# AliaksandrSiarohin/wc-gan

Hardware: AMD Instinct MI355X
Metric: images/sec G+D step, CIFAR-10 ResNet-SN+WC, batch 64 (higher is better)
Workload: dtype f32; 1 GPU; CIFAR-10 ResNet SN uncond + WC (scripts/cifar10_resnet_sn_uncond.sh), batch 64/GPU, training_ratio 5, generator_batch_multiple 2; parallelism=dp1, wc_statistics=per-replica, launch=hipgraph

## Files before the change

include/wc_hip.h:

```cpp
#ifndef WC_HIP_H
#define WC_HIP_H

#include <stddef.h>
#include <stdint.h>

#ifdef __cplusplus
extern "C" {
#endif

#define WC_ABI_VERSION 8

#define WC_OK                 0
#define WC_ERR_NULL          -1
#define WC_ERR_SHAPE         -2
#define WC_ERR_CHANNELS      -3
#define WC_ERR_WORKSPACE     -4
#define WC_ERR_ARG           -5

typedef void* wc_stream_t;

int         wc_abi_version(void);
const char* wc_error_string(int code);

#define WC_CORE_API "wc_stats_f32 wc_factor_f64 wc_color_f32 wc_group_bias_f32 wc_apply_f32 wc_apply_act_f32 " \
// ... 246 lines not shown

#define WC_CONV_HIST_FLOATS (4 * 512 + 16)
#define WC_CONV_HIST_REDO (4 * 512)
int wc_conv_split_hist_f32(const float* x, int64_t n, int relu, void* hi, void* lo, float* scale, float* colsum_partials , int C,
                           float* hist, int bootstrap, wc_stream_t stream);

int wc_conv_split_leaky_f32(const float* x, int64_t n, float negative_slope, void* hi, void* lo, float* scale, void* amax_scratch,
                            float* colsum_partials , int C, wc_stream_t stream);
int wc_conv_split_hist_leaky_f32(const float* x, int64_t n, float negative_slope, void* hi, void* lo, float* scale,
                                 float* colsum_partials , int C, float* hist, int bootstrap, wc_stream_t stream);
int wc_conv_leaky_bwd_f32(float* dx, const float* x, int64_t n, float negative_slope, wc_stream_t stream);

size_t wc_conv_weights_bytes(const wc_conv_geom* g);
int wc_conv_weights_f32(const float* w, int64_t stride_k, int64_t stride_n, int64_t stride_r, int64_t stride_s,
                        int64_t n_elems, const wc_conv_geom* g, void* image, float* scale, void* amax_scratch,
                        const float* known_amax, int known_count, wc_stream_t stream);

int wc_conv_weights_pair_f32(const float* w, int64_t stride_r, int64_t stride_s, int64_t n_elems,
                             int64_t a_stride_k, int64_t a_stride_n, const wc_conv_geom* ga, void* image_a,
                             int64_t b_stride_k, int64_t b_stride_n, const wc_conv_geom* gb, void* image_b,
                             float* scale, void* amax_scratch, const float* known_amax, int known_count,
                             wc_stream_t stream);

size_t wc_conv_workspace_bytes(const wc_conv_geom* g);
int wc_conv_f16x3(const void* xhi, const void* xlo, const float* xscale, const void* wimage, const float* wscale,
                  const float* bias, const void* zero_line, const wc_conv_geom* g, int relu, float* y,
                  void* ws, size_t ws_bytes, wc_stream_t stream);

int wc_conv_res_supported(const wc_conv_geom* g);
int wc_conv_res_f16x3(const void* xhi, const void* xlo, const float* xscale, const void* wimage, const float* wscale,
                      const float* bias, const float* res, const void* zero_line, const wc_conv_geom* g, float* y,
                      void* ws, size_t ws_bytes, wc_stream_t stream);
int wc_conv_block_dx_f32(const float* dx1, const float* x, const float* other, int64_t N, int64_t H, int64_t W, int C, int down,
                         float* out, wc_stream_t stream);

size_t wc_conv_wrw_workspace_bytes(const wc_conv_geom* g);
int wc_conv_wrw_f16x3(const void* xhi, const void* xlo, const float* xscale, const void* ghi, const void* glo,
                      const float* gscale, const void* zero_line, const wc_conv_geom* g, float* dw, int64_t stride_k,
                      int64_t stride_n, int64_t stride_r, int64_t stride_s, void* ws, size_t ws_bytes,
                      wc_stream_t stream);

int    wc_conv_wrw_narrow_supported(int64_t N, int64_t H, int64_t W, int Cin, int Cout, int ksize);
size_t wc_conv_wrw_narrow_workspace_bytes(int64_t N, int64_t H, int64_t W, int Cin, int Cout, int ksize);
int    wc_conv_wrw_narrow_f32(const float* x, const float* gy, int64_t N, int64_t H, int64_t W, int Cin, int Cout, int ksize,
                              float* dw, int64_t stride_k, int64_t stride_n, int64_t stride_r, int64_t stride_s, float* db ,
                              void* ws, size_t ws_bytes, wc_stream_t stream);
// ... 118 lines not shown
```

wc_gan_amd/_lib.py:

```python
from __future__ import annotations

import ctypes
import os
from ctypes import c_float, c_char_p, c_double, c_int, c_int64, c_size_t, c_void_p

_HERE = os.path.dirname(os.path.abspath(__file__))
LIB_PATH = os.path.join(_HERE, "libwc_hip.so")

WC_OK = 0
ABI_VERSION = 8
ERRORS = {-1: "WC_ERR_NULL", -2: "WC_ERR_SHAPE", -3: "WC_ERR_CHANNELS", -4: "WC_ERR_WORKSPACE", -5: "WC_ERR_ARG"}

SIGNATURES = {
    "wc_abi_version": (c_int, []),
    "wc_error_string": (c_char_p, [c_int]),
    "wc_stats_workspace_bytes": (c_size_t, [c_int64, c_int, c_int]),
    "wc_factor_workspace_bytes": (c_size_t, [c_int, c_int]),
    "wc_color_workspace_bytes": (c_size_t, [c_int, c_int]),
    "wc_bwd_reduce_workspace_bytes": (c_size_t, [c_int64, c_int64, c_int, c_int, c_int]),
    "wc_bwd_factor_workspace_bytes": (c_size_t, [c_int, c_int]),
    "wc_apply_workspace_bytes": (c_size_t, [c_int64, c_int64, c_int, c_int]),
    "wc_apply_plan_bytes": (c_size_t, [c_int, c_int]),
    "wc_bwd_apply_workspace_bytes": (c_size_t, [c_int64, c_int64, c_int, c_int]),
    "wc_stats_f32": (c_int, [c_void_p, c_int64, c_int, c_int, c_void_p, c_void_p, c_void_p, c_size_t, c_void_p]),
# ... 102 lines not shown
    "wc_conv_weights_f32": (c_int, [c_void_p, c_int64, c_int64, c_int64, c_int64, c_int64, c_void_p, c_void_p, c_void_p,
                                    c_void_p, c_void_p, c_int, c_void_p]),
    "wc_spectral_norm_amax_offset": (c_size_t, [c_int, c_int]),
    "wc_spectral_norm_error_offset": (c_size_t, [c_int, c_int]),
    "wc_conv_split_hist_f32": (c_int, [c_void_p, c_int64, c_int, c_void_p, c_void_p, c_void_p, c_void_p, c_int, c_void_p, c_int, c_void_p]),
    "wc_conv_split_leaky_f32": (c_int, [c_void_p, c_int64, c_float, c_void_p, c_void_p, c_void_p, c_void_p, c_void_p, c_int, c_void_p]),
    "wc_conv_split_hist_leaky_f32": (c_int, [c_void_p, c_int64, c_float, c_void_p, c_void_p, c_void_p, c_void_p, c_int, c_void_p, c_int, c_void_p]),
    "wc_conv_leaky_bwd_f32": (c_int, [c_void_p, c_void_p, c_int64, c_float, c_void_p]),
    "wc_conv_narrow64_supported": (c_int, [c_int64, c_int64, c_int64, c_int, c_int, c_int]),
    "wc_conv_wrw_narrow64_workspace_bytes": (c_size_t, [c_int64, c_int64, c_int64, c_int, c_int, c_int]),
    "wc_conv_wrw_narrow64_f32": (c_int, [c_void_p, c_void_p, c_int64, c_int64, c_int64, c_int, c_int, c_int, c_void_p, c_int64, c_int64, c_int64,
                                         c_int64, c_void_p, c_void_p, c_size_t, c_void_p]),
    "wc_conv_fwd_narrow_f32": (c_int, [c_void_p, c_void_p, c_int64, c_int64, c_int64, c_int64, c_void_p, c_int64, c_int64, c_int64, c_int, c_int, c_int,
                                       c_int, c_void_p, c_void_p]),
    "wc_conv_wrw_narrow_supported": (c_int, [c_int64, c_int64, c_int64, c_int, c_int, c_int]),
    "wc_conv_wrw_narrow_workspace_bytes": (c_size_t, [c_int64, c_int64, c_int64, c_int, c_int, c_int]),
    "wc_conv_wrw_narrow_f32": (c_int, [c_void_p, c_void_p, c_int64, c_int64, c_int64, c_int, c_int, c_int, c_void_p, c_int64, c_int64, c_int64,
                                       c_int64, c_void_p, c_void_p, c_size_t, c_void_p]),
    "wc_conv_split_colsum_f32": (c_int, [c_void_p, c_int64, c_int, c_void_p, c_void_p, c_void_p, c_void_p, c_void_p, c_int, c_void_p]),
    "wc_conv_wrw_bias_f16x3": (c_int, [c_void_p, c_void_p, c_void_p, c_void_p, c_void_p, c_void_p, c_void_p, c_void_p, c_void_p,
                                       c_int64, c_int64, c_int64, c_int64, c_void_p, c_void_p, c_void_p, c_size_t, c_void_p]),
    "wc_conv_weights_pair_f32": (c_int, [c_void_p, c_int64, c_int64, c_int64, c_int64, c_int64, c_void_p, c_void_p,
                                         c_int64, c_int64, c_void_p, c_void_p, c_void_p, c_void_p, c_void_p, c_int, c_void_p]),
    "wc_conv_wrw_workspace_bytes": (c_size_t, [c_void_p]),
    "wc_conv_wrw_f16x3": (c_int, [c_void_p, c_void_p, c_void_p, c_void_p, c_void_p, c_void_p, c_void_p, c_void_p, c_void_p,
                                  c_int64, c_int64, c_int64, c_int64, c_void_p, c_size_t, c_void_p]),
    "wc_conv_workspace_bytes": (c_size_t, [c_void_p]),
    "wc_conv_f16x3": (c_int, [c_void_p, c_void_p, c_void_p, c_void_p, c_void_p, c_void_p, c_void_p, c_void_p, c_int,
                              c_void_p, c_void_p, c_size_t, c_void_p]),
    "wc_conv_bwd_pair_supported": (c_int, [c_void_p, c_void_p]),
    "wc_conv_bwd_pair_workspace_bytes": (c_size_t, [c_void_p, c_void_p]),
    "wc_conv_bwd_pair_f16x3": (c_int, [c_void_p, c_void_p, c_void_p, c_void_p, c_void_p, c_void_p, c_void_p, c_void_p, c_void_p, c_size_t,
                                       c_void_p, c_void_p, c_void_p, c_void_p, c_void_p, c_int64, c_int64, c_int64, c_int64,
                                       c_void_p, c_void_p, c_void_p, c_size_t, c_void_p]),
    "wc_std_stats_workspace_bytes": (c_size_t, [c_int64, c_int, c_int]),
    "wc_std_stats_f32": (c_int, [c_void_p, c_int64, c_int, c_int, c_void_p, c_void_p, c_void_p, c_size_t, c_void_p]),
    "wc_std_factor_f64": (c_int, [c_void_p, c_void_p, c_int64, c_int, c_int, c_double, c_double, c_int, c_int, c_void_p, c_void_p,
                                  c_void_p, c_void_p, c_int, c_void_p, c_void_p, c_void_p, c_void_p, c_void_p]),
    "wc_std_apply_f32": (c_int, [c_void_p, c_void_p, c_void_p, c_void_p, c_int64, c_int64, c_int, c_int, c_int, c_void_p, c_void_p]),
    "wc_std_bwd_reduce_workspace_bytes": (c_size_t, [c_int64, c_int64, c_int, c_int]),
    "wc_std_bwd_reduce_f32": (c_int, [c_void_p, c_void_p, c_void_p, c_void_p, c_void_p, c_int64, c_int64, c_int, c_int, c_int,
                                      c_void_p, c_void_p, c_void_p, c_size_t, c_void_p]),
    "wc_std_bwd_factor_f64": (c_int, [c_void_p, c_void_p, c_void_p, c_void_p, c_void_p, c_int64, c_int, c_int, c_int,
                                      c_void_p, c_void_p, c_void_p, c_void_p, c_void_p]),
    "wc_std_bwd_apply_f32": (c_int, [c_void_p, c_void_p, c_void_p, c_void_p, c_void_p, c_void_p, c_void_p, c_int64, c_int64, c_int, c_int,
                                     c_int, c_void_p, c_void_p]),
# ... 37 lines not shown


class SnItem(ctypes.Structure):
    _fields_ = [("W", c_void_p), ("u", c_void_p), ("v", c_void_p), ("w_sn", c_void_p), ("sigma", c_void_p),
                ("u_used", c_void_p), ("v_used", c_void_p), ("ws", c_void_p), ("rows", c_int), ("cols", c_int)]


class SnBwdItem(ctypes.Structure):
    _fields_ = [("g", c_void_p), ("w_sn", c_void_p), ("u", c_void_p), ("v", c_void_p), ("sigma", c_void_p),
                ("dW", c_void_p), ("ws", c_void_p), ("rows", c_int), ("cols", c_int)]


class ConvGeom(ctypes.Structure):
    _fields_ = [("N", c_int), ("H", c_int), ("W", c_int), ("Hin", c_int), ("Win", c_int), ("Cin", c_int),
                ("Hout", c_int), ("Wout", c_int), ("Cout", c_int), ("in_stride", c_int), ("out_stride", c_int),
                ("ntaps", c_int), ("nphase", c_int),
                ("dy", (ctypes.c_byte * 16) * 4), ("dx", (ctypes.c_byte * 16) * 4),
                ("off_y", ctypes.c_byte * 4), ("off_x", ctypes.c_byte * 4),
                ("nsrc", (ctypes.c_byte * 16) * 4),
                ("wr", ((ctypes.c_byte * 4) * 16) * 4), ("ws", ((ctypes.c_byte * 4) * 16) * 4),
                ("wcoef", c_float)]


_lib = None


class WcHipError(RuntimeError):
    pass


def shared_gpu_guard(device_count=None) -> bool:
    if "WC_K2_TWO_LAUNCH" in os.environ:
        if os.environ["WC_K2_TWO_LAUNCH"] == "0":
            del os.environ["WC_K2_TWO_LAUNCH"]
        return False
    try:
        ranks = int(os.environ.get("LOCAL_WORLD_SIZE", "1") or 1)
    except ValueError:
        ranks = 1
    if ranks <= 1:
        return False
    if any(os.environ.get(k) for k in ("HIP_VISIBLE_DEVICES", "CUDA_VISIBLE_DEVICES", "ROCR_VISIBLE_DEVICES")):
        return False
    if device_count is None:
        try:
            import torch
# ... 38 lines not shown
```

wc_gan_amd/conv.py:

```python
from __future__ import annotations

import ctypes
import os

import torch
import torch.nn.functional as F

from . import _lib, _state
from .ops import _ptr, _stream

_zero_lines = {}


def _zero_line(device):
    z = _zero_lines.get(device)
    if z is None:
        z = _zero_lines[device] = torch.zeros(64, dtype=torch.uint8, device=device)
    return z


def _plain(r, s):
    return [(r, s)], 1.0


# ... 201 lines not shown
def block_input_gradient(dx1, x, other, down):
    N, H, W, C = dx1.shape
    want = (N, H // 2, W // 2, C) if down else (N, H, W, C)
    if not (dx1.is_contiguous() and x.is_contiguous() and other.is_contiguous() and x.shape == dx1.shape and tuple(other.shape) == want
            and dx1.dtype == x.dtype == other.dtype == torch.float32):
        raise ValueError("block_input_gradient: dense fp32 NHWC tensors, `other` of dx1's shape (at half resolution when down)")
    out = torch.empty_like(dx1)
    _lib.check(_lib.load().wc_conv_block_dx_f32(_ptr(dx1), _ptr(x), _ptr(other), N, H, W, C, 1 if down else 0, _ptr(out), _stream()),
               "wc_conv_block_dx_f32")
    return out


def leaky_backward_(dx, x, slope):
    if not (dx.is_contiguous() and x.is_contiguous() and dx.shape == x.shape and dx.dtype == x.dtype == torch.float32):
        raise ValueError("leaky_backward_: dense fp32 tensors of one shape")
    _lib.check(_lib.load().wc_conv_leaky_bwd_f32(_ptr(dx), _ptr(x), dx.numel(), float(slope), _stream()), "wc_conv_leaky_bwd_f32")
    return dx


def _storage_extent(w):
    return 1 + sum((n - 1) * s for n, s in zip(w.shape, w.stride()))


def weight_image(w, geom, k_axis, n_axis):
    lib = _lib.load()
    nbytes = lib.wc_conv_weights_bytes(ctypes.addressof(geom))
    img = torch.empty(nbytes, dtype=torch.uint8, device=w.device)
    scale = torch.empty(1 + 512, dtype=torch.float32, device=w.device)
    ext = _storage_extent(w)
    if ext != w.numel():
        raise ValueError("weight must be dense")
    known = getattr(w, '_wc_amax', None)
    _lib.check(lib.wc_conv_weights_f32(_ptr(w), w.stride(k_axis), w.stride(n_axis), w.stride(2), w.stride(3), ext,
                                       ctypes.addressof(geom), _ptr(img), _ptr(scale), scale.data_ptr() + 4,
                                       _ptr(known), 0 if known is None else known.numel(), _stream()),
               "wc_conv_weights_f32")
    return img, scale


def weight_image_pair(w, fwd, bwd):
    lib = _lib.load()
    (ga, ka, na), (gb, kb, nb) = fwd, bwd
    img_a = torch.empty(lib.wc_conv_weights_bytes(ctypes.addressof(ga)), dtype=torch.uint8, device=w.device)
    img_b = torch.empty(lib.wc_conv_weights_bytes(ctypes.addressof(gb)), dtype=torch.uint8, device=w.device)
    scale = torch.empty(2 + 512, dtype=torch.float32, device=w.device)
    ext = _storage_extent(w)
    if ext != w.numel():
        raise ValueError("weight must be dense")
    known = getattr(w, '_wc_amax', None)
    _lib.check(lib.wc_conv_weights_pair_f32(_ptr(w), w.stride(2), w.stride(3), ext,
                                            w.stride(ka), w.stride(na), ctypes.addressof(ga), _ptr(img_a),
                                            w.stride(kb), w.stride(nb), ctypes.addressof(gb), _ptr(img_b),
                                            _ptr(scale), scale.data_ptr() + 8, _ptr(known), 0 if known is None else known.numel(),
                                            _stream()), "wc_conv_weights_pair_f32")
    return (img_a, scale[0:1]), (img_b, scale[1:2])


def _cached_image(w, key, geom, k_axis, n_axis):
    return weight_image(w, geom, k_axis, n_axis)


def run(planes, image, geom, bias=None, relu=False, nbytes=None, res=None):
    hi, lo, xs = planes
    img, ws = image
    lib = _lib.load()
    y = torch.empty((geom.N, geom.Hout, geom.Wout, geom.Cout), dtype=torch.float32, device=hi.device)
    if nbytes is None:
        nbytes = lib.wc_conv_workspace_bytes(ctypes.addressof(geom))
    work = torch.empty(nbytes, dtype=torch.uint8, device=hi.device) if nbytes else None
    if res is not None:
        if relu or not (res.is_contiguous() and res.shape == y.shape and res.dtype == torch.float32 and res.device == y.device):
            raise ValueError("run: the residual is a dense fp32 tensor of the output's shape (and there is no ReLU behind it)")
        _lib.check(lib.wc_conv_res_f16x3(_ptr(hi), _ptr(lo), _ptr(xs), _ptr(img), _ptr(ws), _ptr(bias) if bias is not None else None,
                                         _ptr(res), _ptr(_zero_line(hi.device)), ctypes.addressof(geom), _ptr(y),
                                         _ptr(work), nbytes, _stream()), "wc_conv_res_f16x3")
        return y
    _lib.check(lib.wc_conv_f16x3(_ptr(hi), _ptr(lo), _ptr(xs), _ptr(img), _ptr(ws), _ptr(bias) if bias is not None else None,
                                 _ptr(_zero_line(hi.device)), ctypes.addressof(geom), 1 if relu else 0, _ptr(y),
                                 _ptr(work), nbytes, _stream()), "wc_conv_f16x3")
    return y


# ... 58 lines not shown
                                          _ptr(work_dx), plan.bwd_ws,
                                          _ptr(xh), _ptr(xl), _ptr(xs), plan.fwd_ptr, _ptr(dw), w.stride(kf), w.stride(nf), w.stride(2),
                                          w.stride(3), _ptr(colsum), _ptr(db), _ptr(work_dw), plan.wrw_ws, _stream()),
               "wc_conv_bwd_pair_f16x3")
    return dx, dw, db


def takes_planes(shape, wshape, kind):
    class _S:
        pass
    xs, ws = _S(), _S()
    xs.shape, ws.shape = tuple(shape), tuple(wshape)
    p = _plan(kind, xs, ws)
    return bool(p) and p.ok


class _FastConv(torch.autograd.Function):
    @staticmethod
    def forward(ctx, x, w, bias, kind, plan, relu_input=False, handed=None, site=None, leaky=None, residual=None):
        gf, kf, nf = plan.fwd
        planes = handed if handed is not None else split_planes(x, relu=relu_input, site=site, role='x', leaky=leaky)
        ctx.site, ctx.leaky = site, leaky
        if ctx.needs_input_grad[0]:
            img, ctx.bwd_image = weight_image_pair(w, plan.fwd, plan.bwd)
        else:
            img, ctx.bwd_image = weight_image(w, gf, kf, nf), None
        if residual is not None and plan.res and FUSED_RESIDUAL:
            y = run(planes, img, gf, bias, nbytes=plan.fwd_ws, res=residual.contiguous())
        else:
            y = run(planes, img, gf, bias, nbytes=plan.fwd_ws)
            if residual is not None:
                y = y + residual
        ctx.save_for_backward(w, *planes, *((x,) if (relu_input or leaky is not None) else ()))
        ctx.kind, ctx.has_bias, ctx.plan, ctx.relu_input = kind, bias is not None, plan, relu_input
        return y

    @staticmethod
    def backward(ctx, gy):
        w, xh, xl, xs = ctx.saved_tensors[:4]
        kind, plan = ctx.kind, ctx.plan
        gy = gy.contiguous()
        want_db = ctx.has_bias and ctx.needs_input_grad[2]
        fused_db = want_db and ctx.needs_input_grad[1] and _colsum_ok(gy.shape[-1])
        g_planes = split_planes(gy, colsum=fused_db, site=ctx.site, role='g')
        dx = dw = db = None
        paired = ctx.needs_input_grad[0] and ctx.needs_input_grad[1] and ctx.bwd_image is not None and plan.pair
        if paired:
            dx, dw, pdb = backward_pair(g_planes, ctx.bwd_image, (xh, xl, xs), plan, w, colsum=g_planes[3] if fused_db else None)
            if fused_db:
# ... 23 lines not shown


def _one(device):
    t = _ones.get(device)
    if t is None:
        t = torch.ones(1, dtype=torch.float32, device=device)
        if not torch.cuda.is_current_stream_capturing():
            _ones[device] = t
    return t


class _SplitConv(torch.autograd.Function):

    @staticmethod
    def forward(ctx, x, w, bias, plan, st, site=None):
        from . import ops
        ctx.site = site
        gf, kf, nf = plan.fwd
        wf, bf = ops.fold_channel_scale(w, bias, st.scale, st.center)
        img = weight_image(wf, gf, kf, nf)
        ctx.bwd_image = None
        if ctx.needs_input_grad[0]:
            gb, kb, nb = plan.bwd
            ctx.bwd_image = weight_image(w, gb, kb, nb)
        hi, lo = st.planes[0].view(st.shape), st.planes[1].view(st.shape)
        one = _one(hi.device)
        y = run((hi, lo, one), img, gf, bf, nbytes=plan.fwd_ws)
        ctx.save_for_backward(w, hi, lo, one, st.scale, st.center)
        ctx.plan, ctx.has_bias = plan, bias is not None
        return y

    @staticmethod
    def backward(ctx, gy):
        from . import ops
        w, xh, xl, one, scale, center = ctx.saved_tensors
        plan = ctx.plan
        gy = gy.contiguous()
        need_w = ctx.needs_input_grad[1]
        need_b = ctx.has_bias and ctx.needs_input_grad[2]
        fused_db = need_w and _colsum_ok(gy.shape[-1])
        g_planes = split_planes(gy, colsum=fused_db, site=ctx.site, role='g')
        dx = dw = db = None
        paired = ctx.needs_input_grad[0] and need_w and ctx.bwd_image is not None and plan.pair
        if paired:
            dx, D, db = backward_pair(g_planes, ctx.bwd_image, (xh, xl, one), plan, w, colsum=g_planes[3] if fused_db else None)
            if not fused_db:
                db = gy.sum((0, 1, 2))
# ... 174 lines not shown
        return None
    N, H, W, C = xshape
    F1, F2 = w1shape[0], w2shape[0]
    if tuple(w1shape[1:]) != (C, 3, 3) or tuple(w2shape[1:]) != (F1, 3, 3):
        return None
    if down and (H % 2 or W % 2):
        return None
    if wsshape is None:
        if down or F2 != C:
            return None
    elif tuple(wsshape) != (F2, C, 1, 1):
        return None
    if not (_colsum_ok(F1) and _colsum_ok(F2)):
        return None
    out = (N, H // 2, W // 2) if down else (N, H, W)
    p1 = _plan('same', _Shape(xshape), _Shape(w1shape))
    p2 = _plan('down3' if down else 'same', _Shape((N, H, W, F1)), _Shape(w2shape))
    ps = _plan('same', _Shape(out + (C,)), _Shape(wsshape)) if wsshape is not None else None
    if not (p1 and p1.ok and p2 and p2.ok and (wsshape is None or (ps and ps.ok))):
        return None
    return p1, p2, ps


def _images(w, plan, both):
    if both:
        return weight_image_pair(w, plan.fwd, plan.bwd)
    gf, kf, nf = plan.fwd
    return weight_image(w, gf, kf, nf), None


def _layer_gradients(g_planes, fused_db, x_planes, w, plan, bwd_image, need_dx, need_dw):
    cs = g_planes[3] if fused_db else None
    if need_dx and need_dw and bwd_image is not None and plan.pair:
        return backward_pair(g_planes, bwd_image, x_planes, plan, w, colsum=cs)
    dx = dw = db = None
    if need_dx:
        gb, kb, nb = plan.bwd
        image = bwd_image if bwd_image is not None else weight_image(w, gb, kb, nb)
        dx = run(g_planes[:3], image, gb, nbytes=plan.bwd_ws)
    if need_dw:
        gf, kf, nf = plan.fwd
        if fused_db:
            dw, db = weight_gradient(x_planes, g_planes, gf, w, kf, nf, nbytes=plan.wrw_ws, colsum=cs)
        else:
            dw = weight_gradient(x_planes, g_planes, gf, w, kf, nf, nbytes=plan.wrw_ws)
    return dx, dw, db


def _pool2(x):
    return F.avg_pool2d(x.permute(0, 3, 1, 2), 2).permute(0, 2, 3, 1).contiguous()


class _CriticBlock(torch.autograd.Function):
    @staticmethod
    def forward(ctx, x, w1, b1, w2, b2, ws, bs, sites, plans, down):
        conv1, conv2, shortcut = sites
        p1, p2, ps = plans
        need = ctx.needs_input_grad
        need_h = need[0] or need[1] or need[2]
        x_pl = split_planes(x, relu=True, site=conv1, role='x')
        img1, bimg1 = _images(w1, p1, need[0])
        h = run(x_pl, img1, p1.fwd[0], b1, nbytes=p1.fwd_ws)
        h_pl = split_planes(h, relu=True, site=conv2, role='x')
        img2, bimg2 = _images(w2, p2, need_h)
        s, s_pl, bimgs = x, (), None
        if ws is not None:
            s_pl = split_planes(_pool2(x) if down else x, site=shortcut, role='x')
            imgs, bimgs = _images(ws, ps, need[0])
            s = run(s_pl, imgs, ps.fwd[0], bs, nbytes=ps.fwd_ws)
        if p2.res and FUSED_RESIDUAL:
            y = run(h_pl, img2, p2.fwd[0], b2, nbytes=p2.fwd_ws, res=s)
        else:
            y = run(h_pl, img2, p2.fwd[0], b2, nbytes=p2.fwd_ws) + s
        ctx.save_for_backward(x, h, w1, w2, *x_pl, *h_pl, *s_pl, *((ws,) if ws is not None else ()))
        ctx.sites, ctx.plans, ctx.down = sites, plans, down
        ctx.images = (bimg1, bimg2, bimgs)
        ctx.has_bias = (b1 is not None, b2 is not None, bs is not None)
        ctx.mark_non_differentiable(h)
        ctx.set_materialize_grads(False)
        return y, h

    @staticmethod
    def backward(ctx, g, _gh):
        saved = ctx.saved_tensors
        x, h, w1, w2 = saved[:4]
        x_pl, h_pl = saved[4:7], saved[7:10]
        conv1, conv2, shortcut = ctx.sites
        p1, p2, ps = ctx.plans
        bimg1, bimg2, bimgs = ctx.images
        need = ctx.needs_input_grad
        need_h = need[0] or need[1] or need[2]
# ... 45 lines not shown
```

wc_gan_amd/csrc/wc_conv.hip:

```cpp
#include "wc_common.h"
#include "../../include/wc_hip.h"
#include <stdlib.h>


namespace {

constexpr int kMaxTaps = 16, kMaxPhase = 4;

struct ConvArgs {
    const _Float16* xhi; const _Float16* xlo;
    const _Float16* zero;
    const char* wimg;
    const float* xscale; const float* wscale;
    const float* bias;
    float* y;
    int N, H, W, Hin, Win, Cin, Cout, in_stride, ntaps, nphase, Hout, Wout, out_stride, relu;
    unsigned magHW, shHW, magW, shW;
    int ksplit; float* partial;
    signed char dy[kMaxPhase][kMaxTaps], dx[kMaxPhase][kMaxTaps];
    signed char offy[kMaxPhase], offx[kMaxPhase];
};

__device__ __forceinline__ void lds_dma16(const void* g, unsigned lds)
{
    unsigned keep;
// ... 532 lines not shown
            const float* src = base + a.r[ph][tap][m] * a.sr + a.s[ph][tap][m] * a.ss;
            #pragma unroll
            for (int j = 0; j < 8; ++j) acc8[j] += src[(k0 + j) * a.sk];
        }
        const float cs = a.coef * sc;
        f16x8 h, l;
        #pragma unroll
        for (int j = 0; j < 8; ++j) {
            const float v = acc8[j] * cs;
            h[j] = (_Float16)v; l[j] = (_Float16)(v - (float)h[j]);
        }
        char* dst = a.img + (((((int64_t)(ph * a.ntaps + tap) * nchunk + ch) * nblk + nb) * 2 + ks) * 2) * 1024 + lane * 16;
        *reinterpret_cast<f16x8*>(dst) = h;
        *reinterpret_cast<f16x8*>(dst + 1024) = l;
    }
}

__global__ __launch_bounds__(256) void conv_weights_kernel(WeightArgs a) { conv_weights_body(a, blockIdx.x, gridDim.x); }

__global__ __launch_bounds__(256) void conv_weights_pair_kernel(WeightArgs a, WeightArgs b, int blocks_a)
{
    if ((int)blockIdx.x < blocks_a) conv_weights_body(a, blockIdx.x, blocks_a);
    else conv_weights_body(b, blockIdx.x - blocks_a, gridDim.x - blocks_a);
}

struct WrwOperand {
    const _Float16* hi; const _Float16* lo;
    int Hp, Wp, C, stride;
    signed char dy[kMaxPhase][kMaxTaps], dx[kMaxPhase][kMaxTaps];
};

struct WrwArgs {
    WrwOperand A, B;
    const _Float16* zero;
    float* partial;
    int N, H, W, ntaps, nphase;
    unsigned magHW, shHW, magW, shW;
    int nchunks, cps;
};

typedef short s16x4v __attribute__((__vector_size__(4 * sizeof(short))));

__device__ __forceinline__ f16x8 tr_read8(const char* block, int lane_off)
{
    auto p = (__attribute__((address_space(3))) s16x4v*)((__attribute__((address_space(3))) char*)(block + lane_off));
    auto q = (__attribute__((address_space(3))) s16x4v*)((__attribute__((address_space(3))) char*)(block + lane_off + 256));
// ... 610 lines not shown
    return (int)hipGetLastError();
}

int wc_conv_weights_pair_f32(const float* w, int64_t stride_r, int64_t stride_s, int64_t n_elems,
                             int64_t a_stride_k, int64_t a_stride_n, const wc_conv_geom* ga, void* image_a,
                             int64_t b_stride_k, int64_t b_stride_n, const wc_conv_geom* gb, void* image_b,
                             float* scale, void* amax_scratch, const float* known_amax, int known_count, wc_stream_t stream)
{
    hipStream_t st = (hipStream_t)stream;
    if (!w || !ga || !gb || !image_a || !image_b || !scale || (!amax_scratch && !known_amax) || n_elems <= 0) return WC_ERR_ARG;
    if (known_amax && (known_count < 1 || known_count > 4096)) return WC_ERR_ARG;
    if (!known_amax) hipLaunchKernelGGL(conv_absmax_kernel, dim3(kAmaxBlocks), dim3(256), 0, st, w, n_elems / 4, n_elems, (float*)amax_scratch);
    const float* amax = known_amax ? known_amax : (const float*)amax_scratch;
    const int cnt = known_amax ? known_count : kAmaxBlocks;
    WeightArgs a, b;
    int rc = fill_weight_args(a, w, a_stride_k, a_stride_n, stride_r, stride_s, n_elems, ga, image_a, scale, amax, cnt);
    if (rc != WC_OK) return rc;
    rc = fill_weight_args(b, w, b_stride_k, b_stride_n, stride_r, stride_s, n_elems, gb, image_b, scale + 1, amax, cnt);
    if (rc != WC_OK) return rc;
    if (a.bound_mul != b.bound_mul) return WC_ERR_ARG;
    const int blocks_a = grid_for((int64_t)ga->nphase * ga->ntaps * (ga->Cin >> 5) * (ga->Cout >> 5) * 128);
    const int blocks_b = grid_for((int64_t)gb->nphase * gb->ntaps * (gb->Cin >> 5) * (gb->Cout >> 5) * 128);
    hipLaunchKernelGGL(conv_weights_pair_kernel, dim3(blocks_a + blocks_b), dim3(256), 0, st, a, b, blocks_a);
    return (int)hipGetLastError();
}

int wc_conv_supported(const wc_conv_geom* g)
{
    if (!g) return 0;
    if (g->ntaps < 1 || g->ntaps > kMaxTaps || g->nphase < 1 || g->nphase > kMaxPhase) return 0;
    if ((g->Cin & 31) || (g->Cout & 63)) return 0;
    const int64_t M = (int64_t)g->N * g->H * g->W;
    if (M <= 0 || (M & 127) || M > (int64_t)1 << 31) return 0;
    if ((int64_t)g->N * g->Hin * g->Win > (int64_t)1 << 31) return 0;
    if (g->W < 2 || g->H < 1) return 0;
    return 1;
}

constexpr int kKsplitMaxWgs = 96;
constexpr int kKsplitTargetWgs = 256;
constexpr int kWrwTargetWgs = 512;

static int conv_ksplit(const wc_conv_geom* g)
{
    const int64_t M = (int64_t)g->N * g->H * g->W;
    const bool wide = (g->Cout % 256) == 0;
// ... 393 lines not shown
```

wc_gan_amd/discriminator.py:

```python
from __future__ import annotations

from functools import partial

import torch
import torch.nn as nn
import torch.nn.functional as F

from .generator import Conv2D, create_norm, to_nchw_view, to_nhwc


def downsample2x(x):
    return to_nhwc(F.avg_pool2d(to_nchw_view(x), 2))


class ResBlockDown(nn.Module):
    def __init__(self, in_ch, nfilters, resample, name, norm, conv_layer, is_first):
        super().__init__()
        assert resample in ('DOWN', 'SAME')
        self.resample, self.is_first = resample, is_first
        self.bn1 = norm(axis=-1, name=name + '.bn1', channels=in_ch)
        self.conv1 = conv_layer(in_ch, nfilters, (3, 3), name=name + '.conv1')
        self.bn2 = norm(axis=-1, name=name + '.bn2', channels=nfilters)
        self.conv2 = conv_layer(nfilters, nfilters, (3, 3), name=name + '.conv2')
        self.has_shortcut = (in_ch != nfilters) or resample == 'DOWN'
# ... 85 lines not shown
        self.dropout = nn.Dropout(dropout) if dropout else None
        emb_dim = ch
        if arch == 'dcgan':
            h, w = (int(v) for v in input_hw)
            for rs in resamples:
                if rs == 'DOWN':
                    if h % 2 or w % 2:
                        raise ValueError(f"arch='dcgan': a DOWN block halves a {h} x {w} grid")
                    h, w = h // 2, w // 2
            if type == 'PROJECTIVE' and h * w != 1:
                raise ValueError(f"arch='dcgan' with type='PROJECTIVE' needs a 1 x 1 final grid (the embedding has block_sizes[-1] = {ch} "
                                 f"dimensions, the flattened features {h} x {w} x {ch}); no shipped recipe combines them")
            ch = h * w * ch
        self.out = dense(ch, 1)
        if type == 'AC_GAN':
            self.cls_out = nn.Linear(ch, number_of_classes)
            nn.init.xavier_uniform_(self.cls_out.weight); nn.init.zeros_(self.cls_out.bias)
        elif type == 'PROJECTIVE':
            self.emb = emb(number_of_classes, emb_dim)

    def forward(self, x, cls=None):
        from .spectral import prepare_spectral
        prepare_spectral(self)
        y = x
        for blk in self.blocks:
            y = blk(y, cls)
        if self.arch == 'dcgan':
            y = F.leaky_relu(y, LEAKY_SLOPE).flatten(1)
        else:
            y = F.relu(y)
            y = y.sum(dim=(1, 2)) if self.sum_pool else y.mean(dim=(1, 2))
        if self.dropout is not None:
            y = self.dropout(y)
        out = self.out(y)
        if self.type == 'AC_GAN':
            return out, self.cls_out(y)
        if self.type == 'PROJECTIVE':
            out = out + (self.emb(cls.reshape(-1).long()) * y).sum(dim=1, keepdim=True)
        return out


def make_discriminator(input_image_shape=(32, 32, 3), input_cls_shape=(1,), block_sizes=(128, 128, 128, 128),
                       resamples=('DOWN', 'DOWN', 'SAME', 'SAME'), number_of_classes=10,
                       type='AC_GAN', norm='n', after_norm='n', spectral=False,
                       fully_diff_spectral=False, spectral_iterations=1, conv_singular=True,
                       sum_pool=False, dropout=False, arch='res', filters_emb=10):
    assert arch in ('res', 'dcgan')
    assert type in [None, 'AC_GAN', 'PROJECTIVE']
    if spectral and conv_singular:
# ... 28 lines not shown
```

Measured before the change: 3812 images/sec.

## Batch discriminator conv weight-image builds into one kernel launch per forward

At the start of each discriminator forward, all per-layer f16x3 weight-image conversions (and any needed absmax sweeps) are built together in one or a few batched kernel launches. This replaces the many small per-layer launches. Which layers and geometries are needed is learned on a first recording pass keyed by input shape and grad/training state, and individual layers then pick up their precomputed images. The aim is to cut launch count and tiny-kernel overhead inside the graph. The cost is extra bookkeeping, and the log is invalidated whenever the recorded and actual requests diverge.

```diff
diff --git a/include/wc_hip.h b/include/wc_hip.h
--- a/include/wc_hip.h
+++ b/include/wc_hip.h
@@ -292,6 +292,18 @@
                              float* scale, void* amax_scratch, const float* known_amax, int known_count,
                              wc_stream_t stream);
 
+typedef struct {
+    const float* w; int64_t stride_k, stride_n, stride_r, stride_s, n_elems;
+    const wc_conv_geom* g; void* image; float* scale;
+    const float* amax; int amax_count; int pair_of;
+} wc_conv_weights_job;
+int wc_conv_weights_batch_f32(const wc_conv_weights_job* jobs, int count, wc_stream_t stream);
+int wc_conv_weights_batch_launches(const wc_conv_weights_job* jobs, int count);
+
+#define WC_CONV_ABSMAX_FLOATS 512
+typedef struct { const float* x; int64_t n; float* partial; } wc_conv_absmax_job;
+int wc_conv_absmax_batch_f32(const wc_conv_absmax_job* jobs, int count, wc_stream_t stream);
+
 size_t wc_conv_workspace_bytes(const wc_conv_geom* g);
 int wc_conv_f16x3(const void* xhi, const void* xlo, const float* xscale, const void* wimage, const float* wscale,
                   const float* bias, const void* zero_line, const wc_conv_geom* g, int relu, float* y,
diff --git a/wc_gan_amd/_lib.py b/wc_gan_amd/_lib.py
--- a/wc_gan_amd/_lib.py
+++ b/wc_gan_amd/_lib.py
@@ -148,6 +148,9 @@
                                        c_int64, c_int64, c_int64, c_int64, c_void_p, c_void_p, c_void_p, c_size_t, c_void_p]),
     "wc_conv_weights_pair_f32": (c_int, [c_void_p, c_int64, c_int64, c_int64, c_int64, c_int64, c_void_p, c_void_p,
                                          c_int64, c_int64, c_void_p, c_void_p, c_void_p, c_void_p, c_void_p, c_int, c_void_p]),
+    "wc_conv_weights_batch_f32": (c_int, [c_void_p, c_int, c_void_p]),
+    "wc_conv_weights_batch_launches": (c_int, [c_void_p, c_int]),
+    "wc_conv_absmax_batch_f32": (c_int, [c_void_p, c_int, c_void_p]),
     "wc_conv_wrw_workspace_bytes": (c_size_t, [c_void_p]),
     "wc_conv_wrw_f16x3": (c_int, [c_void_p, c_void_p, c_void_p, c_void_p, c_void_p, c_void_p, c_void_p, c_void_p, c_void_p,
                                   c_int64, c_int64, c_int64, c_int64, c_void_p, c_size_t, c_void_p]),
@@ -231,6 +234,18 @@
                 ("wcoef", c_float)]
 
 
+class ConvWeightsJob(ctypes.Structure):
+    _fields_ = [("w", c_void_p), ("stride_k", c_int64), ("stride_n", c_int64), ("stride_r", c_int64), ("stride_s", c_int64),
+                ("n_elems", c_int64), ("g", c_void_p), ("image", c_void_p), ("scale", c_void_p), ("amax", c_void_p),
+                ("amax_count", c_int), ("pair_of", c_int)]
+
+
+class ConvAbsmaxJob(ctypes.Structure):
+    _fields_ = [("x", c_void_p), ("n", c_int64), ("partial", c_void_p)]
+
+
+ABSMAX_FLOATS = 512
+
 _lib = None
 
 
diff --git a/wc_gan_amd/conv.py b/wc_gan_amd/conv.py
--- a/wc_gan_amd/conv.py
+++ b/wc_gan_amd/conv.py
@@ -247,7 +247,11 @@
     return 1 + sum((n - 1) * s for n, s in zip(w.shape, w.stride()))
 
 
-def weight_image(w, geom, k_axis, n_axis):
+def weight_image(w, geom, k_axis, n_axis, site=None):
+    if site is not None:
+        got = _pick_up(site, w, ((geom, k_axis, n_axis),))
+        if got is not None:
+            return got
     lib = _lib.load()
     nbytes = lib.wc_conv_weights_bytes(ctypes.addressof(geom))
     img = torch.empty(nbytes, dtype=torch.uint8, device=w.device)
@@ -263,7 +267,11 @@
     return img, scale
 
 
-def weight_image_pair(w, fwd, bwd):
+def weight_image_pair(w, fwd, bwd, site=None):
+    if site is not None:
+        got = _pick_up(site, w, (fwd, bwd))
+        if got is not None:
+            return got
     lib = _lib.load()
     (ga, ka, na), (gb, kb, nb) = fwd, bwd
     img_a = torch.empty(lib.wc_conv_weights_bytes(ctypes.addressof(ga)), dtype=torch.uint8, device=w.device)
@@ -283,6 +291,139 @@
 
 def _cached_image(w, key, geom, k_axis, n_axis):
     return weight_image(w, geom, k_axis, n_axis)
+
+
+BATCH_IMAGES = True
+_recording = None
+_prepared = None
+
+
+def pass_key(root, x):
+    return (tuple(x.shape), torch.is_grad_enabled(), bool(x.requires_grad), root.training,
+            tuple(p.requires_grad for p in root.parameters()))
+
+
+def _own_weight(site):
+    conv = getattr(site, 'conv', None)
+    if conv is None:
+        return None
+    if hasattr(conv, 'normalized_weight'):
+        ready = getattr(conv, '_w_ready', None)
+        if ready is None or ready[1] != conv.weight._version or ready[2] != conv.training:
+            return None
+        return ready[0]
+    return conv.weight
+
+
+def _same_geoms(a, b):
+    return len(a) == len(b) and all(p[0] is q[0] and p[1] == q[1] and p[2] == q[2] for p, q in zip(a, b))
+
+
+def build_images(requests):
+    lib = _lib.load()
+    dev = requests[0][0].device
+    sizes = [[lib.wc_conv_weights_bytes(ctypes.addressof(g[0])) for g in geoms] for _, geoms in requests]
+    njobs = sum(len(s) for s in sizes)
+    images = torch.empty(sum(sum(s) for s in sizes), dtype=torch.uint8, device=dev)
+    scales = torch.empty(njobs, dtype=torch.float32, device=dev)
+    jobs = (_lib.ConvWeightsJob * njobs)()
+    measure = []
+    for w, _ in requests:
+        ext = _storage_extent(w)
+        if ext != w.numel():
+            raise ValueError("weight must be dense")
+        if getattr(w, '_wc_amax', None) is None and not (ext <= 32768 and ext % 4 == 0 and w.data_ptr() % 16 == 0):
+            measure.append(w)
+    partials = None
+    if measure:
+        partials = torch.empty(len(measure) * _lib.ABSMAX_FLOATS, dtype=torch.float32, device=dev)
+        sweeps = (_lib.ConvAbsmaxJob * len(measure))()
+        for i, w in enumerate(measure):
+            sweeps[i].x, sweeps[i].n, sweeps[i].partial = w.data_ptr(), w.numel(), partials.data_ptr() + 4 * _lib.ABSMAX_FLOATS * i
+        _lib.check(lib.wc_conv_absmax_batch_f32(ctypes.addressof(sweeps), len(measure), _stream()), "wc_conv_absmax_batch_f32")
+    out, j, off, m = [], 0, 0, 0
+    for (w, geoms), nbytes in zip(requests, sizes):
+        known = getattr(w, '_wc_amax', None)
+        if known is not None:
+            amax, count = known.data_ptr(), known.numel()
+        elif m < len(measure) and measure[m] is w:
+            amax, count = partials.data_ptr() + 4 * _lib.ABSMAX_FLOATS * m, _lib.ABSMAX_FLOATS
+            m += 1
+        else:
+            amax, count = None, 0
+        res = []
+        for i, ((g, k_axis, n_axis), nb) in enumerate(zip(geoms, nbytes)):
+            job = jobs[j]
+            job.w, job.n_elems, job.g = w.data_ptr(), w.numel(), ctypes.addressof(g)
+            job.stride_k, job.stride_n, job.stride_r, job.stride_s = w.stride(k_axis), w.stride(n_axis), w.stride(2), w.stride(3)
+            job.image, job.scale = images.data_ptr() + off, scales.data_ptr() + 4 * j
+            job.amax, job.amax_count, job.pair_of = amax, count, (j - 1 if i else -1)
+            res.append((images[off:off + nb], scales[j:j + 1]))
+            j += 1
+            off += nb
+        out.append(tuple(res))
+    _lib.check(lib.wc_conv_weights_batch_f32(ctypes.addressof(jobs), njobs, _stream()), "wc_conv_weights_batch_f32")
+    return out
+
+
+def _clear_images(root):
+    for site in root.__dict__.get('_wc_image_sites', ()):
+        site._wc_images = None
+    root._wc_image_sites = ()
+
+
+def prepare_images(root, key):
+    global _recording, _prepared
+    _clear_images(root)
+    _recording = _prepared = None
+    if not BATCH_IMAGES:
+        return
+    logs = root.__dict__.get('_wc_image_logs')
+    if logs is None:
+        logs = root._wc_image_logs = {}
+    log = logs.get(key)
+    if log is None:
+        _recording = (root, key, [])
+        return
+    _prepared = [root, key, False]
+    requests, sites = [], []
+    for site, geoms in log:
+        w = _own_weight(site)
+        if w is not None and w.dtype == torch.float32 and w.dim() == 4:
+            requests.append((w, geoms))
+            sites.append(site)
+    if not requests:
+        return
+    for site, (w, geoms), images in zip(sites, requests, build_images(requests)):
+        if site.__dict__.get('_wc_images') is None:
+            site._wc_images = []
+        site._wc_images.append((w, geoms, images if len(geoms) > 1 else images[0]))
+    root._wc_image_sites = tuple(sites)
+
+
+def _pick_up(site, w, geoms):
+    recs = site.__dict__.get('_wc_images')
+    if recs:
+        for i, (rw, rgeoms, images) in enumerate(recs):
+            if rw is w and _same_geoms(rgeoms, geoms):
+                del recs[i]
+                return images
+    if _recording is not None:
+        _recording[2].append((site, tuple(geoms)))
+    elif _prepared is not None:
+        _prepared[2] = True
+    return None
+
+
+def finish_images(root):
+    global _recording, _prepared
+    if _recording is not None and _recording[0] is root:
+        root._wc_image_logs[_recording[1]] = _recording[2]
+    elif _prepared is not None and _prepared[0] is root:
+        if _prepared[2] or any(site.__dict__.get('_wc_images') for site in root.__dict__.get('_wc_image_sites', ())):
+            root._wc_image_logs.pop(_prepared[1], None)
+    _recording = _prepared = None
+    _clear_images(root)
 
 
 def run(planes, image, geom, bias=None, relu=False, nbytes=None, res=None):
@@ -387,9 +528,9 @@
         planes = handed if handed is not None else split_planes(x, relu=relu_input, site=site, role='x', leaky=leaky)
         ctx.site, ctx.leaky = site, leaky
         if ctx.needs_input_grad[0]:
-            img, ctx.bwd_image = weight_image_pair(w, plan.fwd, plan.bwd)
+            img, ctx.bwd_image = weight_image_pair(w, plan.fwd, plan.bwd, site=site)
         else:
-            img, ctx.bwd_image = weight_image(w, gf, kf, nf), None
+            img, ctx.bwd_image = weight_image(w, gf, kf, nf, site=site), None
         if residual is not None and plan.res and FUSED_RESIDUAL:
             y = run(planes, img, gf, bias, nbytes=plan.fwd_ws, res=residual.contiguous())
         else:
@@ -459,7 +600,7 @@
         ctx.bwd_image = None
         if ctx.needs_input_grad[0]:
             gb, kb, nb = plan.bwd
-            ctx.bwd_image = weight_image(w, gb, kb, nb)
+            ctx.bwd_image = weight_image(w, gb, kb, nb, site=site)
         hi, lo = st.planes[0].view(st.shape), st.planes[1].view(st.shape)
         one = _one(hi.device)
         y = run((hi, lo, one), img, gf, bf, nbytes=plan.fwd_ws)
@@ -680,11 +821,11 @@
     return p1, p2, ps
 
 
-def _images(w, plan, both):
+def _images(w, plan, both, site=None):
     if both:
-        return weight_image_pair(w, plan.fwd, plan.bwd)
+        return weight_image_pair(w, plan.fwd, plan.bwd, site=site)
     gf, kf, nf = plan.fwd
-    return weight_image(w, gf, kf, nf), None
+    return weight_image(w, gf, kf, nf, site=site), None
 
 
 def _layer_gradients(g_planes, fused_db, x_planes, w, plan, bwd_image, need_dx, need_dw):
@@ -717,14 +858,14 @@
         need = ctx.needs_input_grad
         need_h = need[0] or need[1] or need[2]
         x_pl = split_planes(x, relu=True, site=conv1, role='x')
-        img1, bimg1 = _images(w1, p1, need[0])
+        img1, bimg1 = _images(w1, p1, need[0], conv1)
         h = run(x_pl, img1, p1.fwd[0], b1, nbytes=p1.fwd_ws)
         h_pl = split_planes(h, relu=True, site=conv2, role='x')
-        img2, bimg2 = _images(w2, p2, need_h)
+        img2, bimg2 = _images(w2, p2, need_h, conv2)
         s, s_pl, bimgs = x, (), None
         if ws is not None:
             s_pl = split_planes(_pool2(x) if down else x, site=shortcut, role='x')
-            imgs, bimgs = _images(ws, ps, need[0])
+            imgs, bimgs = _images(ws, ps, need[0], shortcut)
             s = run(s_pl, imgs, ps.fwd[0], bs, nbytes=ps.fwd_ws)
         if p2.res and FUSED_RESIDUAL:
             y = run(h_pl, img2, p2.fwd[0], b2, nbytes=p2.fwd_ws, res=s)
diff --git a/wc_gan_amd/csrc/wc_conv.hip b/wc_gan_amd/csrc/wc_conv.hip
--- a/wc_gan_amd/csrc/wc_conv.hip
+++ b/wc_gan_amd/csrc/wc_conv.hip
@@ -1,6 +1,7 @@
 #include "wc_common.h"
 #include "../../include/wc_hip.h"
 #include <stdlib.h>
+#include <string.h>
 
 
 namespace {
@@ -579,6 +580,77 @@
 {
     if ((int)blockIdx.x < blocks_a) conv_weights_body(a, blockIdx.x, blocks_a);
     else conv_weights_body(b, blockIdx.x - blocks_a, gridDim.x - blocks_a);
+}
+
+constexpr int kBatchJobs = 16, kBatchTables = 6;
+constexpr int kBatchBlocks = 16384;
+
+struct BatchJob {
+    const float* w; const float* amax; float* scale_out; char* img;
+    int64_t sk, sn, sr, ss, n4;
+    int K, Nn;
+    float coef, bound_mul;
+    int amax_count, table;
+};
+struct BatchTable {
+    int ntaps, nphase;
+    signed char nsrc[kMaxPhase][kMaxTaps];
+    unsigned char rs[kMaxPhase][kMaxTaps][4];
+};
+struct WeightBatch {
+    BatchJob job[kBatchJobs];
+    BatchTable table[kBatchTables];
+    int first[kBatchJobs + 1];
+    int count;
+};
+static_assert(sizeof(WeightBatch) <= 4096, "the batch travels in the kernel arguments");
+
+__global__ __launch_bounds__(256) void conv_weights_batch_kernel(WeightBatch q)
+{
+    __shared__ WeightArgs a;
+    int i = 0;
+    while (i + 1 < q.count && (int)blockIdx.x >= q.first[i + 1]) ++i;
+    const BatchJob& j = q.job[i];
+    const BatchTable& t = q.table[j.table];
+    if (threadIdx.x == 0) {
+        a.w = j.w; a.sk = j.sk; a.sn = j.sn; a.sr = j.sr; a.ss = j.ss;
+        a.amax = j.amax; a.scale_out = j.scale_out; a.img = j.img;
+        a.K = j.K; a.Nn = j.Nn; a.ntaps = t.ntaps; a.nphase = t.nphase;
+        a.n4 = j.n4; a.coef = j.coef; a.bound_mul = j.bound_mul; a.amax_count = j.amax_count;
+    }
+    for (int e = threadIdx.x; e < kMaxPhase * kMaxTaps * 4; e += 256) {
+        const int p = e / (kMaxTaps * 4), tp = (e >> 2) % kMaxTaps, m = e & 3;
+        const unsigned char v = t.rs[p][tp][m];
+        a.r[p][tp][m] = (signed char)(v & 3);
+        a.s[p][tp][m] = (signed char)(v >> 2);
+        if (m == 0) a.nsrc[p][tp] = t.nsrc[p][tp];
+    }
+    __syncthreads();
+    conv_weights_body(a, (int)blockIdx.x - q.first[i], q.first[i + 1] - q.first[i]);
+}
+
+constexpr int kAbsmaxJobs = 32;
+struct AbsmaxJob { const float* x; int64_t n; float* partial; };
+struct AbsmaxBatch { AbsmaxJob job[kAbsmaxJobs]; };
+
+__global__ __launch_bounds__(256) void conv_absmax_batch_kernel(AbsmaxBatch q)
+{
+    __shared__ float red[4];
+    const AbsmaxJob& j = q.job[blockIdx.x / kAmaxBlocks];
+    const int bid = blockIdx.x % kAmaxBlocks;
+    const float* __restrict__ x = j.x;
+    const int64_t n4 = j.n >> 2;
+    float m = 0.f;
+    for (int64_t i = bid * 256 + threadIdx.x; i < n4; i += (int64_t)kAmaxBlocks * 256) {
+        const f32x4 v = *reinterpret_cast<const f32x4*>(x + 4 * i);
+        m = fmaxf(fmaxf(m, fabsf(v[0])), fmaxf(fabsf(v[1]), fmaxf(fabsf(v[2]), fabsf(v[3]))));
+    }
+    if (bid == 0 && threadIdx.x == 0) for (int64_t i = 4 * n4; i < j.n; ++i) m = fmaxf(m, fabsf(x[i]));
+    #pragma unroll
+    for (int o = 32; o > 0; o >>= 1) m = fmaxf(m, __shfl_xor(m, o));
+    if ((threadIdx.x & 63) == 0) red[threadIdx.x >> 6] = m;
+    __syncthreads();
+    if (threadIdx.x == 0) j.partial[bid] = fmaxf(fmaxf(red[0], red[1]), fmaxf(red[2], red[3]));
 }
 
 struct WrwOperand {
@@ -1235,6 +1307,111 @@
     const int blocks_a = grid_for((int64_t)ga->nphase * ga->ntaps * (ga->Cin >> 5) * (ga->Cout >> 5) * 128);
     const int blocks_b = grid_for((int64_t)gb->nphase * gb->ntaps * (gb->Cin >> 5) * (gb->Cout >> 5) * 128);
     hipLaunchKernelGGL(conv_weights_pair_kernel, dim3(blocks_a + blocks_b), dim3(256), 0, st, a, b, blocks_a);
+    return (int)hipGetLastError();
+}
+
+static void fill_batch_table(BatchTable& t, const WeightArgs& a)
+{
+    memset(&t, 0, sizeof(t));
+    t.ntaps = a.ntaps; t.nphase = a.nphase;
+    for (int p = 0; p < a.nphase; ++p)
+        for (int k = 0; k < a.ntaps; ++k) {
+            t.nsrc[p][k] = a.nsrc[p][k];
+            for (int m = 0; m < a.nsrc[p][k]; ++m) t.rs[p][k][m] = (unsigned char)(a.r[p][k][m] | (a.s[p][k][m] << 2));
+        }
+}
+
+static int check_weights_job(const wc_conv_weights_job& j, WeightArgs& a)
+{
+    if (!j.w || !j.g || !j.image || !j.scale) return WC_ERR_NULL;
+    if (j.n_elems <= 0) return WC_ERR_ARG;
+    if (j.amax) { if (j.amax_count < 1 || j.amax_count > 4096) return WC_ERR_ARG; }
+    else if (j.n_elems > 32768 || (j.n_elems & 3) || ((uintptr_t)j.w & 15)) return WC_ERR_ARG;
+    const int rc = fill_weight_args(a, j.w, j.stride_k, j.stride_n, j.stride_r, j.stride_s, j.n_elems, j.g, j.image, j.scale, j.amax,
+                                    j.amax ? j.amax_count : 0);
+    if (rc != WC_OK) return rc;
+    for (int p = 0; p < a.nphase; ++p)
+        for (int k = 0; k < a.ntaps; ++k)
+            for (int m = 0; m < a.nsrc[p][k]; ++m)
+                if (a.r[p][k][m] < 0 || a.r[p][k][m] > 3 || a.s[p][k][m] < 0 || a.s[p][k][m] > 3) return WC_ERR_ARG;
+    return WC_OK;
+}
+
+static int weights_batch(const wc_conv_weights_job* jobs, int count, bool launch, hipStream_t st, int* launches)
+{
+    if (!jobs) return WC_ERR_NULL;
+    if (count <= 0) return WC_ERR_SHAPE;
+    *launches = 0;
+    WeightArgs a, b;
+    for (int i = 0; i < count; ++i) {
+        int rc = check_weights_job(jobs[i], a);
+        if (rc != WC_OK) return rc;
+        const int p = jobs[i].pair_of;
+        if (p < 0) continue;
+        if (p >= i) return WC_ERR_ARG;
+        rc = check_weights_job(jobs[p], b);
+        if (rc != WC_OK) return rc;
+        if (jobs[p].w != jobs[i].w || jobs[p].amax != jobs[i].amax || jobs[p].amax_count != jobs[i].amax_count
+            || jobs[p].n_elems != jobs[i].n_elems || a.bound_mul != b.bound_mul) return WC_ERR_ARG;
+    }
+    for (int c0 = 0; c0 < count;) {
+        WeightBatch q;
+        memset(&q, 0, sizeof(q));
+        int take = 0, blocks = 0, ntab = 0;
+        while (c0 + take < count && take < kBatchJobs) {
+            const wc_conv_weights_job& j = jobs[c0 + take];
+            (void)check_weights_job(j, a);
+            BatchTable t;
+            fill_batch_table(t, a);
+            int ti = 0;
+            while (ti < ntab && memcmp(&q.table[ti], &t, sizeof(t)) != 0) ++ti;
+            const int nb = grid_for((int64_t)a.nphase * a.ntaps * (a.K >> 5) * (a.Nn >> 5) * 128);
+            if (take > 0 && (ti == kBatchTables || blocks + nb > kBatchBlocks)) break;
+            if (ti == ntab) q.table[ntab++] = t;
+            BatchJob& o = q.job[take];
+            o.w = a.w; o.amax = a.amax; o.scale_out = a.scale_out; o.img = a.img;
+            o.sk = a.sk; o.sn = a.sn; o.sr = a.sr; o.ss = a.ss; o.n4 = a.n4;
+            o.K = a.K; o.Nn = a.Nn; o.coef = a.coef; o.bound_mul = a.bound_mul; o.amax_count = a.amax_count; o.table = ti;
+            q.first[take] = blocks;
+            blocks += nb; ++take;
+        }
+        q.first[take] = blocks;
+        q.count = take;
+        if (launch) hipLaunchKernelGGL(conv_weights_batch_kernel, dim3(blocks), dim3(256), 0, st, q);
+        ++*launches;
+        c0 += take;
+    }
+    return launch ? (int)hipGetLastError() : WC_OK;
+}
+
+int wc_conv_weights_batch_f32(const wc_conv_weights_job* jobs, int count, wc_stream_t stream)
+{
+    int launches;
+    return weights_batch(jobs, count, true, (hipStream_t)stream, &launches);
+}
+
+int wc_conv_weights_batch_launches(const wc_conv_weights_job* jobs, int count)
+{
+    int launches = 0;
+    const int rc = weights_batch(jobs, count, false, nullptr, &launches);
+    return rc != WC_OK ? rc : launches;
+}
+
+int wc_conv_absmax_batch_f32(const wc_conv_absmax_job* jobs, int count, wc_stream_t stream)
+{
+    if (!jobs) return WC_ERR_NULL;
+    if (count <= 0) return WC_ERR_SHAPE;
+    for (int i = 0; i < count; ++i) {
+        if (!jobs[i].x || !jobs[i].partial) return WC_ERR_NULL;
+        if (jobs[i].n <= 0 || ((uintptr_t)jobs[i].x & 15)) return WC_ERR_ARG;
+    }
+    for (int c0 = 0; c0 < count; c0 += kAbsmaxJobs) {
+        AbsmaxBatch q;
+        memset(&q, 0, sizeof(q));
+        const int take = count - c0 < kAbsmaxJobs ? count - c0 : kAbsmaxJobs;
+        for (int i = 0; i < take; ++i) q.job[i] = AbsmaxJob{jobs[c0 + i].x, jobs[c0 + i].n, jobs[c0 + i].partial};
+        hipLaunchKernelGGL(conv_absmax_batch_kernel, dim3(take * kAmaxBlocks), dim3(256), 0, (hipStream_t)stream, q);
+    }
     return (int)hipGetLastError();
 }
 
diff --git a/wc_gan_amd/discriminator.py b/wc_gan_amd/discriminator.py
--- a/wc_gan_amd/discriminator.py
+++ b/wc_gan_amd/discriminator.py
@@ -131,9 +131,17 @@
     def forward(self, x, cls=None):
         from .spectral import prepare_spectral
         prepare_spectral(self)
-        y = x
-        for blk in self.blocks:
-            y = blk(y, cls)
+        from . import conv as fc
+        batch = torch.is_tensor(x) and x.is_cuda
+        if batch:
+            fc.prepare_images(self, fc.pass_key(self, x))
+        try:
+            y = x
+            for blk in self.blocks:
+                y = blk(y, cls)
+        finally:
+            if batch:
+                fc.finish_images(self)
         if self.arch == 'dcgan':
             y = F.leaky_relu(y, LEAKY_SLOPE).flatten(1)
         else:
```

Result: faster. 3856 images/sec (median of 6 runs) (+1.1%).
